# ai4ce/V2X-Sim

Measured on AMD Instinct MI355X. Metric: BEV frames/sec, V2VNet 5-agent detection (256x256 BEV), higher is better.
Workload: dtype bf16

## Files before the change

### v2x-sim_amd/csrc/conv_tail.hip

```cpp
#include "conv_stream.h"
#include <cstdlib>

typedef const __attribute__((address_space(1))) void *gptr_tl_t;
typedef __attribute__((address_space(3))) void *lptr_tl_t;

typedef unsigned int u32x2_tl_t __attribute__((ext_vector_type(2)));
typedef __attribute__((address_space(3))) u32x2_tl_t lds_u2_t;

static __device__ __attribute__((aligned(64))) unsigned int g_zero_page_tail[16];

struct TailArgs {
    const uint16_t *in;
    int in_cstride, in_coff;
    int N, H, W;
    const uint16_t *wA;
    const float *scA, *shA;
    int reluA;
    const uint16_t *wB;
    const float *scB, *shB;
    int reluB;
    const uint16_t *w2;
    const float *sc2, *sh2;
    int split;
    float *out, *out2;
    int out_cstride, out_coff, out2_cstride;
    int tiles_x, tiles_y, n_tiles;
    int xcd_walk;
};

namespace tail {
constexpr int TH = 8, TW = 32;
constexpr int MH = TH + 2, MW = TW + 2;
constexpr int IH = TH + 4, IW = TW + 4;
constexpr int NMID = MH * MW;
constexpr int WA_BYTES = 36 * 32 * 16;
constexpr int WB_BYTES = 36 * 64 * 16;
constexpr int IN_BYTES = IH * IW * 64;
constexpr int IN_PIECES = IN_BYTES / 1024;
constexpr int PPW = (IN_PIECES + 3) / 4;
constexpr int MID_BYTES = NMID * 64;
constexpr int GRP_BYTES = IN_BYTES + MID_BYTES;
constexpr int OFF_GRP = WA_BYTES + WB_BYTES;
constexpr int OFF_DUMMY = OFF_GRP + 2 * GRP_BYTES;
constexpr int OFF_TAB = OFF_DUMMY + 1024;
constexpr int SMEM = OFF_TAB + 288 * 4;
static_assert(IN_BYTES % 1024 == 0 && SMEM <= 160 * 1024, "LDS map");
__device__ __forceinline__ int swz4(int slot, int x) { return slot ^ ((x >> 1) & 3); }
}

__global__ __launch_bounds__(512) __attribute__((amdgpu_waves_per_eu(2, 2))) void conv3x3_tail_kernel(const TailArgs a) {
    using namespace tail;
    extern __shared__ __attribute__((aligned(16))) char smem[];
    const int tid = threadIdx.x;
    const int lane = tid & 63;
    const int wave8 = __builtin_amdgcn_readfirstlane(tid >> 6);
    const int grp = wave8 >> 2, wave = wave8 & 3;
    const int fj = lane & 15, fq = lane >> 4;
    char *s_wA = smem, *s_wB = smem + WA_BYTES;
    char *s_in = smem + OFF_GRP + grp * GRP_BYTES, *s_mid = s_in + IN_BYTES;

    for (int off = wave8 * 1024; off < WA_BYTES + WB_BYTES; off += 8192) {
        const char *src = off < WA_BYTES ? reinterpret_cast<const char *>(a.wA) + off : reinterpret_cast<const char *>(a.wB) + (off - WA_BYTES);
        __builtin_amdgcn_global_load_lds((gptr_tl_t)(src + lane * 16), (lptr_tl_t)(smem + off), 16, 0, 0);
    }
    bf16x8_t w2f[3][2];
#pragma unroll
    for (int i2 = 0; i2 < 3; ++i2)
#pragma unroll
        for (int s = 0; s < 2; ++s) w2f[i2][s] = *reinterpret_cast<const bf16x8_t *>(a.w2 + (size_t)(i2 * 16 + fj) * 64 + s * 32 + fq * 8);
    float *s_tab = reinterpret_cast<float *>(smem + OFF_TAB);
    for (int i = tid; i < 288; i += 512) {
        float v;
        if (i < 32) v = a.scA[i];
        else if (i < 64) v = a.shA[i - 32];
        else if (i < 128) v = a.scB[i - 64];
        else if (i < 192) v = a.shB[i - 128];
        else if (i < 240) v = a.sc2[i - 192];
        else v = a.sh2[i - 240];
        s_tab[i] = v;
    }
    const uint32_t floorA = a.reluA ? 0u : 0x80008000u, floorB = a.reluB ? 0u : 0x80008000u;
#pragma unroll
    for (int i = 0; i < 3; ++i) asm volatile("" ::"v"(w2f[i][0]), "v"(w2f[i][1]));

    const int r0 = wave < 2 ? 3 * wave : 6 + 2 * (wave - 2);
    int body_off[2][3];
#pragma unroll
    for (int sg = 0; sg < 2; ++sg)
#pragma unroll
        for (int kx = 0; kx < 3; ++kx) {
            const int col = 1 + 16 * sg + fj + kx;
            body_off[sg][kx] = (col * 4 + swz4(fq, col)) * 16;
        }
    int hr, hc, hvalid;
    {
        const int q = (wave == 3 ? 16 : 0) + fj;
        const int qc = q < 20 ? q : 19;
        hc = qc < 10 ? 0 : MW - 1;
        hr = qc < 10 ? qc : qc - 10;
        hvalid = (wave >= 2 && q < 20) ? 1 : 0;
    }
    const int txy = a.tiles_x * a.tiles_y;
    auto tile_coords = [&](int tile, int &n, int &ty, int &tx) {
        n = tile / txy;
        const int r = tile - n * txy;
        ty = r / a.tiles_x;
        tx = r - ty * a.tiles_x;
    };
    unsigned woff[PPW];
#pragma unroll
    for (int u = 0; u < PPW; ++u) {
        const int sidx = (wave + 4 * u) * 64 + lane;
        const int pix = sidx >> 2, phys = sidx & 3;
        const int pr = pix / IW, pcx = pix - pr * IW;
        woff[u] = (unsigned)(pr * a.W + pcx) * (unsigned)a.in_cstride + (unsigned)(swz4(phys, pcx) * 8);
    }
    auto load_window = [&](int tile) {
        int n, ty, tx;
        tile_coords(tile, n, ty, tx);
        const bool interior = ty > 0 && ty + 1 < a.tiles_y && tx > 0 && tx + 1 < a.tiles_x;
        if (interior) {
            const uint16_t *base = a.in + (size_t)((n * a.H + ty * TH - 2) * a.W + tx * TW - 2) * a.in_cstride + a.in_coff;
#pragma unroll
            for (int u = 0; u < PPW; ++u) {
                const int piece = wave + 4 * u;
                char *dst = piece < IN_PIECES ? s_in + piece * 1024 : smem + OFF_DUMMY;
                __builtin_amdgcn_global_load_lds((gptr_tl_t)(piece < IN_PIECES ? (const void *)(base + woff[u]) : (const void *)g_zero_page_tail), (lptr_tl_t)dst, 16, 0, 0);
            }
            return;
        }
        const int ln = fresh_lane();
#pragma unroll
        for (int u = 0; u < PPW; ++u) {
            const int piece = wave + 4 * u;
            const int sidx = piece * 64 + ln;
            const int pix = sidx >> 2, phys = sidx & 3;
            const int pr = pix / IW, pcx = pix - pr * IW;
            const int y = ty * TH - 2 + pr, x = tx * TW - 2 + pcx;
            const bool ok = piece < IN_PIECES && (unsigned)y < (unsigned)a.H && (unsigned)x < (unsigned)a.W;
            const unsigned off = (unsigned)((n * a.H + y) * a.W + x) * (unsigned)a.in_cstride + (unsigned)(a.in_coff + swz4(phys, pcx) * 8);
            char *dst = piece < IN_PIECES ? s_in + piece * 1024 : smem + OFF_DUMMY;
            __builtin_amdgcn_global_load_lds((gptr_tl_t)(ok ? (const void *)(a.in + off) : (const void *)g_zero_page_tail), (lptr_tl_t)dst, 16, 0, 0);
        }
    };

    const int n_pairs = (a.n_tiles + 1) >> 1;
    const v2x_tile_walk walk = v2x_xcd_tile_walk(n_pairs, a.xcd_walk);
    int pair_i = walk.first;
    {
        const int tile = 2 * pair_i + grp;
        if (pair_i < walk.end && tile < a.n_tiles) load_window(tile);
    }
    asm volatile("s_waitcnt vmcnt(0)" ::: "memory");
    __syncthreads();
    if (grp == 1) __builtin_amdgcn_s_barrier();

    for (; pair_i < walk.end; pair_i += walk.step) {
        const int tile = 2 * pair_i + grp;
        const bool has = tile < a.n_tiles;
        const int next_pair = pair_i + walk.step;
        const int next = 2 * next_pair + grp;
        const bool has_next = next_pair < walk.end && next < a.n_tiles;
        int n = 0, ty = 0, tx = 0;
        tile_coords(has ? tile : 0, n, ty, tx);

        if (has) {
            f32x4_t acc[6][2];
#pragma unroll
            for (int t = 0; t < 6; ++t)
#pragma unroll
                for (int i = 0; i < 2; ++i) acc[t][i] = (f32x4_t){0.f, 0.f, 0.f, 0.f};
            const char *wrow = s_in + r0 * (IW * 64);
#pragma unroll
            for (int kx = 0; kx < 3; ++kx) {
                bf16x8_t A[3][2], Bb[4][2], X[3];
#pragma unroll
                for (int ky = 0; ky < 3; ++ky)
#pragma unroll
                    for (int i = 0; i < 2; ++i) A[ky][i] = *reinterpret_cast<const bf16x8_t *>(s_wA + (((ky * 3 + kx) * 4 + fq) * 32 + i * 16 + fj) * 16);
#pragma unroll
                for (int rr = 0; rr < 4; ++rr)
#pragma unroll
                    for (int sg = 0; sg < 2; ++sg) Bb[rr][sg] = *reinterpret_cast<const bf16x8_t *>(wrow + rr * (IW * 64) + body_off[sg][kx]);
                if (wave < 2) {
#pragma unroll
                    for (int sg = 0; sg < 2; ++sg) X[sg] = *reinterpret_cast<const bf16x8_t *>(wrow + 4 * (IW * 64) + body_off[sg][kx]);
                    X[2] = X[1];
                } else {
                    const int col = hc + kx;
#pragma unroll
                    for (int ky = 0; ky < 3; ++ky) X[ky] = *reinterpret_cast<const bf16x8_t *>(s_in + (((hr + ky) * IW + col) * 4 + swz4(fq, col)) * 16);
                }
                __builtin_amdgcn_sched_barrier(0);
#pragma unroll
                for (int ky = 0; ky < 3; ++ky) {
#pragma unroll
                    for (int j = 0; j < 2; ++j)
#pragma unroll
                        for (int sg = 0; sg < 2; ++sg)
#pragma unroll
                            for (int i = 0; i < 2; ++i)
                                acc[2 * j + sg][i] = __builtin_amdgcn_mfma_f32_16x16x32_bf16(A[ky][i], Bb[j + ky][sg], acc[2 * j + sg][i], 0, 0, 0);
                    if (wave < 2) {
#pragma unroll
                        for (int sg = 0; sg < 2; ++sg)
#pragma unroll
                            for (int i = 0; i < 2; ++i)
                                acc[4 + sg][i] = __builtin_amdgcn_mfma_f32_16x16x32_bf16(A[ky][i], ky == 2 ? X[sg] : Bb[2 + ky][sg], acc[4 + sg][i], 0, 0, 0);
                    } else {
#pragma unroll
                        for (int i = 0; i < 2; ++i) acc[4][i] = __builtin_amdgcn_mfma_f32_16x16x32_bf16(A[ky][i], X[ky], acc[4][i], 0, 0, 0);
                    }
                }
                __builtin_amdgcn_sched_barrier(0);
            }
            float4 scA[2], shA[2];
#pragma unroll
            for (int i = 0; i < 2; ++i) {
                scA[i] = lds_ld4((lds_cf_t *)s_tab + i * 16 + fq * 4);
                shA[i] = lds_ld4((lds_cf_t *)s_tab + 32 + i * 16 + fq * 4);
            }
            auto emit = [&](const f32x4_t (&v)[2], int r, int c, bool keep, bool inside) __attribute__((always_inline)) {
#pragma unroll
                for (int i = 0; i < 2; ++i) {
                    uint2 o;
                    o.x = v2x_relu_bf16x2_floor(pack_bf16x2(v[i][0] * scA[i].x + shA[i].x, v[i][1] * scA[i].y + shA[i].y), floorA);
                    o.y = v2x_relu_bf16x2_floor(pack_bf16x2(v[i][2] * scA[i].z + shA[i].z, v[i][3] * scA[i].w + shA[i].w), floorA);
                    o.x = inside ? o.x : 0u;
                    o.y = inside ? o.y : 0u;
                    if (keep) *(lds_u2_t *)(s_mid + ((r * MW + c) * 4 + swz4(i * 2 + (fq >> 1), c)) * 16 + (fq & 1) * 8) = (u32x2_tl_t){o.x, o.y};
                }
            };
#pragma unroll
            for (int j = 0; j < 3; ++j) {
                if (j == 2 && wave >= 2) break;
                const int r = r0 + j;
                const int y = ty * TH - 1 + r;
                const bool inside = (unsigned)y < (unsigned)a.H;
#pragma unroll
                for (int sg = 0; sg < 2; ++sg) emit(acc[2 * j + sg], r, 1 + 16 * sg + fj, true, inside);
            }
            if (wave >= 2) {
                const int y = ty * TH - 1 + hr, x = tx * TW - 1 + hc;
                emit(acc[4], hr, hc, hvalid != 0, (unsigned)y < (unsigned)a.H && (unsigned)x < (unsigned)a.W);
            }
        }
        asm volatile("s_waitcnt lgkmcnt(0)" ::: "memory");
        __builtin_amdgcn_sched_barrier(0);
        __builtin_amdgcn_s_barrier();
        __builtin_amdgcn_sched_barrier(0);
        if (has_next) load_window(next);

        if (has) {
            f32x4_t acc[4][4];
#pragma unroll
            for (int i = 0; i < 4; ++i)
#pragma unroll
                for (int f = 0; f < 4; ++f) acc[i][f] = (f32x4_t){0.f, 0.f, 0.f, 0.f};
#pragma unroll
            for (int kx = 0; kx < 3; ++kx) {
                bf16x8_t A[2][4], B[8];
#pragma unroll
                for (int rr = 0; rr < 4; ++rr)
#pragma unroll
                    for (int ch = 0; ch < 2; ++ch) {
                        const int pr = 2 * wave + rr, pc = ch * 16 + fj + kx;
                        B[rr * 2 + ch] = *reinterpret_cast<const bf16x8_t *>(s_mid + ((pr * MW + pc) * 4 + swz4(fq, pc)) * 16);
                    }
#pragma unroll
                for (int i = 0; i < 4; ++i) A[0][i] = *reinterpret_cast<const bf16x8_t *>(s_wB + ((kx * 4 + fq) * 64 + i * 16 + fj) * 16);
#pragma unroll
                for (int ky = 0; ky < 3; ++ky) {
                    __builtin_amdgcn_sched_barrier(0);
                    if (ky < 2) {
#pragma unroll
                        for (int i = 0; i < 4; ++i)
                            A[(ky + 1) & 1][i] = *reinterpret_cast<const bf16x8_t *>(s_wB + ((((ky + 1) * 3 + kx) * 4 + fq) * 64 + i * 16 + fj) * 16);
                    }
                    __builtin_amdgcn_sched_barrier(0);
#pragma unroll
                    for (int i = 0; i < 4; ++i)
#pragma unroll
                        for (int f = 0; f < 4; ++f)
                            acc[i][f] = __builtin_amdgcn_mfma_f32_16x16x32_bf16(A[ky & 1][i], B[((f >> 1) + ky) * 2 + (f & 1)], acc[i][f], 0, 0, 0);
                }
                __builtin_amdgcn_sched_barrier(0);
            }
            float4 scB[4], shB[4], s2v[3], t2v[3];
#pragma unroll
            for (int i = 0; i < 4; ++i) {
                const int kappa = 32 * (i >> 1) + 8 * fq + 4 * (i & 1);
                scB[i] = lds_ld4((lds_cf_t *)s_tab + 64 + kappa);
                shB[i] = lds_ld4((lds_cf_t *)s_tab + 128 + kappa);
            }
#pragma unroll
            for (int i2 = 0; i2 < 3; ++i2) {
                s2v[i2] = lds_ld4((lds_cf_t *)s_tab + 192 + i2 * 16 + fq * 4);
                t2v[i2] = lds_ld4((lds_cf_t *)s_tab + 240 + i2 * 16 + fq * 4);
            }
#pragma unroll
            for (int f = 0; f < 4; ++f) {
                bf16x8_t hb[2];
#pragma unroll
                for (int s = 0; s < 2; ++s) {
                    float h[8];
#pragma unroll
                    for (int half = 0; half < 2; ++half) {
                        const int i = 2 * s + half;
                        h[half * 4 + 0] = acc[i][f][0] * scB[i].x + shB[i].x;
                        h[half * 4 + 1] = acc[i][f][1] * scB[i].y + shB[i].y;
                        h[half * 4 + 2] = acc[i][f][2] * scB[i].z + shB[i].z;
                        h[half * 4 + 3] = acc[i][f][3] * scB[i].w + shB[i].w;
                    }
                    uint4 p;
                    p.x = v2x_relu_bf16x2_floor(pack_bf16x2(h[0], h[1]), floorB);
                    p.y = v2x_relu_bf16x2_floor(pack_bf16x2(h[2], h[3]), floorB);
                    p.z = v2x_relu_bf16x2_floor(pack_bf16x2(h[4], h[5]), floorB);
                    p.w = v2x_relu_bf16x2_floor(pack_bf16x2(h[6], h[7]), floorB);
                    hb[s] = __builtin_bit_cast(bf16x8_t, p);
                }
                const int y = ty * TH + 2 * wave + (f >> 1), x = tx * TW + (f & 1) * 16 + fj;
                const uint32_t pix = (uint32_t)((n * a.H + y) * a.W + x);
                float *p1 = a.out + (size_t)pix * a.out_cstride + a.out_coff + fq * 4;
                float *p2 = a.out2 + (size_t)pix * a.out2_cstride + fq * 4 - a.split;
                float *p0 = (fq * 4 >= a.split) ? p2 : p1;
#pragma unroll
                for (int i2 = 0; i2 < 3; ++i2) {
                    f32x4_t d = (f32x4_t){0.f, 0.f, 0.f, 0.f};
#pragma unroll
                    for (int s = 0; s < 2; ++s) d = __builtin_amdgcn_mfma_f32_16x16x32_bf16(w2f[i2][s], hb[s], d, 0, 0, 0);
                    const float4 s2 = s2v[i2], t2 = t2v[i2];
                    const float v0 = d[0] * s2.x + t2.x, v1 = d[1] * s2.y + t2.y, v2 = d[2] * s2.z + t2.z, v3 = d[3] * s2.w + t2.w;
                    *reinterpret_cast<float4 *>(i2 == 0 ? p0 : p2 + i2 * 16) = make_float4(v0, v1, v2, v3);
                }
            }
        }
        if (has) asm volatile("s_waitcnt vmcnt(12)" ::: "memory");
        else asm volatile("s_waitcnt vmcnt(0)" ::: "memory");
        __builtin_amdgcn_sched_barrier(0);
        __builtin_amdgcn_s_barrier();
        __builtin_amdgcn_sched_barrier(0);
    }
    if (grp == 0) __builtin_amdgcn_s_barrier();
}


static int tail_launch(const TailArgs &a, hipStream_t s) {
    const int n_pairs = (a.n_tiles + 1) / 2;
    int grid = v2x_num_cus();
    if (grid > n_pairs) grid = n_pairs;
    return v2x_launch<conv3x3_tail_kernel>("conv3x3_tail_kernel", dim3(grid), dim3(512), tail::SMEM, s, a);
}

int v2x_conv_tail_dispatch(const v2x_conv_desc *first, const v2x_conv_desc *second, hipStream_t stream) {
    V2X_REQUIRE(first->ksize == 3 && first->stride == 1 && first->pad == 1 && first->w_layout == 1 && first->C0 == 32 && first->C1 == 0 && first->Cout == 32 &&
                    first->Cout2 == 0 && first->epilogue == V2X_EPI_BF16 && first->up0 == 0 && first->in_format == 0,
                "v2x_conv2d_pair (tail form): the first layer must be a halo-packed 3x3 stride-1 32 -> 32 bf16 layer on a bf16 NHWC input");
    V2X_REQUIRE(second->ksize == 3 && second->stride == 1 && second->pad == 1 && second->w_layout == 1 && second->C0 == 32 && second->C1 == 0 &&
                    second->Cout == 64 && second->Cout2 == 48 && second->epilogue == V2X_EPI_F32 && second->up0 == 0 && second->split > 0 &&
                    second->split % 4 == 0 && second->split <= 12 && second->relu2 == 0,
                "v2x_conv2d_pair (tail form): the second layer must be the fused heads (3x3 32 -> 64 chained with a 1x1 -> 48 without ReLU, fp32 outputs split at 4, 8 or 12 channels)");
    V2X_REQUIRE(first->in0 && first->weight && first->scale && first->shift && second->weight && second->scale && second->shift && second->weight2 &&
                    second->scale2 && second->shift2 && second->out && second->out2,
                "v2x_conv2d_pair (tail form): null pointer");
    V2X_REQUIRE(first->N == second->N && first->H == second->H && first->W == second->W, "v2x_conv2d_pair (tail form): extents differ");
    V2X_REQUIRE(first->N >= 0 && first->H > 0 && first->W > 0 && first->H % tail::TH == 0 && first->W % tail::TW == 0,
                "v2x_conv2d_pair (tail form): H %% 8 == 0 and W %% 32 == 0 required (H=%d W=%d)", first->H, first->W);
    V2X_REQUIRE((long long)first->N * first->H * first->W < (1ll << 27), "v2x_conv2d_pair (tail form): N*H*W must stay below 2^27 (32-bit element offsets)");
    V2X_REQUIRE(second->out_cstride >= second->split + second->out_coff && second->out_cstride % 4 == 0 && second->out_coff % 4 == 0 &&
                    second->out2_cstride >= 48 - second->split && second->out2_cstride % 4 == 0 && (reinterpret_cast<uintptr_t>(second->out) & 15) == 0 &&
                    (reinterpret_cast<uintptr_t>(second->out2) & 15) == 0,
                "v2x_conv2d_pair (tail form): bad output views (16-byte stores)");
    if (first->N == 0) return V2X_OK;
    TailArgs a;
    a.in = first->in0;
    a.in_cstride = 32;
    a.in_coff = 0;
    a.N = first->N;
    a.H = first->H;
    a.W = first->W;
    a.wA = first->weight;
    a.scA = first->scale;
    a.shA = first->shift;
    a.reluA = first->relu;
    a.wB = second->weight;
    a.scB = second->scale;
    a.shB = second->shift;
    a.reluB = second->relu;
    a.w2 = second->weight2;
    a.sc2 = second->scale2;
    a.sh2 = second->shift2;
    a.split = second->split;
    a.out = reinterpret_cast<float *>(second->out);
    a.out2 = reinterpret_cast<float *>(second->out2);
    a.out_cstride = second->out_cstride;
    a.out_coff = second->out_coff;
    a.out2_cstride = second->out2_cstride;
    a.tiles_x = a.W / tail::TW;
    a.tiles_y = a.H / tail::TH;
    a.n_tiles = a.N * a.tiles_x * a.tiles_y;
    a.xcd_walk = v2x_tune(V2X_TUNE_HALO_XCD);
    return tail_launch(a, stream);
}
```

Before: 6510.

## Walk vertical tile strips with a ring buffer to reuse fused-conv intermediate rows

The fused two-layer 3x3 tail kernel now walks whole vertical strips of tiles instead of independent 8x32 tiles. The intermediate (first-layer) rows sit in a rotating LDS ring, so each step loads and computes only 8 new input rows and 8 new mid rows rather than recomputing the 2-row halo. This removes redundant first-layer MFMA work and halo input loads. In exchange there is a priming step per strip and fewer independent work units (N*tiles_x strip pairs), which may reduce load balance across CUs.

```diff
diff --git a/v2x-sim_amd/csrc/conv_tail.hip b/v2x-sim_amd/csrc/conv_tail.hip
--- a/v2x-sim_amd/csrc/conv_tail.hip
+++ b/v2x-sim_amd/csrc/conv_tail.hip
@@ -31,12 +31,12 @@
 namespace tail {
 constexpr int TH = 8, TW = 32;
 constexpr int MH = TH + 2, MW = TW + 2;
-constexpr int IH = TH + 4, IW = TW + 4;
+constexpr int IH = TH + 2, IW = TW + 4;
 constexpr int NMID = MH * MW;
 constexpr int WA_BYTES = 36 * 32 * 16;
 constexpr int WB_BYTES = 36 * 64 * 16;
-constexpr int IN_BYTES = IH * IW * 64;
-constexpr int IN_PIECES = IN_BYTES / 1024;
+constexpr int IN_PIECES = (IH * IW * 64 + 1023) / 1024;
+constexpr int IN_BYTES = IN_PIECES * 1024;
 constexpr int PPW = (IN_PIECES + 3) / 4;
 constexpr int MID_BYTES = NMID * 64;
 constexpr int GRP_BYTES = IN_BYTES + MID_BYTES;
@@ -83,7 +83,7 @@
 #pragma unroll
     for (int i = 0; i < 3; ++i) asm volatile("" ::"v"(w2f[i][0]), "v"(w2f[i][1]));
 
-    const int r0 = wave < 2 ? 3 * wave : 6 + 2 * (wave - 2);
+    const int r0 = 2 + 2 * wave;
     int body_off[2][3];
 #pragma unroll
     for (int sg = 0; sg < 2; ++sg)
@@ -92,20 +92,10 @@
             const int col = 1 + 16 * sg + fj + kx;
             body_off[sg][kx] = (col * 4 + swz4(fq, col)) * 16;
         }
-    int hr, hc, hvalid;
-    {
-        const int q = (wave == 3 ? 16 : 0) + fj;
-        const int qc = q < 20 ? q : 19;
-        hc = qc < 10 ? 0 : MW - 1;
-        hr = qc < 10 ? qc : qc - 10;
-        hvalid = (wave >= 2 && q < 20) ? 1 : 0;
-    }
-    const int txy = a.tiles_x * a.tiles_y;
-    auto tile_coords = [&](int tile, int &n, int &ty, int &tx) {
-        n = tile / txy;
-        const int r = tile - n * txy;
-        ty = r / a.tiles_x;
-        tx = r - ty * a.tiles_x;
+    const int hc = fj < 8 ? 0 : MW - 1, hr = 2 + (fj & 7);
+    auto strip_coords = [&](int strip, int &n, int &tx) {
+        n = strip / a.tiles_x;
+        tx = strip - n * a.tiles_x;
     };
     unsigned woff[PPW];
 #pragma unroll
@@ -115,12 +105,12 @@
         const int pr = pix / IW, pcx = pix - pr * IW;
         woff[u] = (unsigned)(pr * a.W + pcx) * (unsigned)a.in_cstride + (unsigned)(swz4(phys, pcx) * 8);
     }
-    auto load_window = [&](int tile) {
-        int n, ty, tx;
-        tile_coords(tile, n, ty, tx);
-        const bool interior = ty > 0 && ty + 1 < a.tiles_y && tx > 0 && tx + 1 < a.tiles_x;
+    auto load_window = [&](int strip, int ty) {
+        int n, tx;
+        strip_coords(strip, n, tx);
+        const bool interior = ty >= 0 && ty + 1 < a.tiles_y && tx > 0 && tx + 1 < a.tiles_x;
         if (interior) {
-            const uint16_t *base = a.in + (size_t)((n * a.H + ty * TH - 2) * a.W + tx * TW - 2) * a.in_cstride + a.in_coff;
+            const uint16_t *base = a.in + (size_t)((n * a.H + ty * TH) * a.W + tx * TW - 2) * a.in_cstride + a.in_coff;
 #pragma unroll
             for (int u = 0; u < PPW; ++u) {
                 const int piece = wave + 4 * u;
@@ -136,41 +126,41 @@
             const int sidx = piece * 64 + ln;
             const int pix = sidx >> 2, phys = sidx & 3;
             const int pr = pix / IW, pcx = pix - pr * IW;
-            const int y = ty * TH - 2 + pr, x = tx * TW - 2 + pcx;
-            const bool ok = piece < IN_PIECES && (unsigned)y < (unsigned)a.H && (unsigned)x < (unsigned)a.W;
+            const int y = ty * TH + pr, x = tx * TW - 2 + pcx;
+            const bool ok = piece < IN_PIECES && pr < IH && (unsigned)y < (unsigned)a.H && (unsigned)x < (unsigned)a.W;
             const unsigned off = (unsigned)((n * a.H + y) * a.W + x) * (unsigned)a.in_cstride + (unsigned)(a.in_coff + swz4(phys, pcx) * 8);
             char *dst = piece < IN_PIECES ? s_in + piece * 1024 : smem + OFF_DUMMY;
             __builtin_amdgcn_global_load_lds((gptr_tl_t)(ok ? (const void *)(a.in + off) : (const void *)g_zero_page_tail), (lptr_tl_t)dst, 16, 0, 0);
         }
     };
 
-    const int n_pairs = (a.n_tiles + 1) >> 1;
+    const int n_strips = a.N * a.tiles_x;
+    const int n_pairs = (n_strips + 1) >> 1;
     const v2x_tile_walk walk = v2x_xcd_tile_walk(n_pairs, a.xcd_walk);
     int pair_i = walk.first;
-    {
-        const int tile = 2 * pair_i + grp;
-        if (pair_i < walk.end && tile < a.n_tiles) load_window(tile);
-    }
+    int ty = -1, ring = 2;
+    if (pair_i < walk.end && 2 * pair_i + grp < n_strips) load_window(2 * pair_i + grp, -1);
     asm volatile("s_waitcnt vmcnt(0)" ::: "memory");
     __syncthreads();
     if (grp == 1) __builtin_amdgcn_s_barrier();
 
-    for (; pair_i < walk.end; pair_i += walk.step) {
-        const int tile = 2 * pair_i + grp;
-        const bool has = tile < a.n_tiles;
-        const int next_pair = pair_i + walk.step;
-        const int next = 2 * next_pair + grp;
-        const bool has_next = next_pair < walk.end && next < a.n_tiles;
-        int n = 0, ty = 0, tx = 0;
-        tile_coords(has ? tile : 0, n, ty, tx);
+    while (pair_i < walk.end) {
+        const int strip = 2 * pair_i + grp;
+        const bool has = strip < n_strips;
+        const bool last = ty + 1 == a.tiles_y;
+        const int next_pair = last ? pair_i + walk.step : pair_i;
+        const int next_ty = last ? -1 : ty + 1;
+        const bool has_next = next_pair < walk.end && 2 * next_pair + grp < n_strips;
+        int n = 0, tx = 0;
+        strip_coords(has ? strip : 0, n, tx);
 
         if (has) {
-            f32x4_t acc[6][2];
-#pragma unroll
-            for (int t = 0; t < 6; ++t)
+            f32x4_t acc[5][2];
+#pragma unroll
+            for (int t = 0; t < 5; ++t)
 #pragma unroll
                 for (int i = 0; i < 2; ++i) acc[t][i] = (f32x4_t){0.f, 0.f, 0.f, 0.f};
-            const char *wrow = s_in + r0 * (IW * 64);
+            const char *wrow = s_in + (r0 - 2) * (IW * 64);
 #pragma unroll
             for (int kx = 0; kx < 3; ++kx) {
                 bf16x8_t A[3][2], Bb[4][2], X[3];
@@ -182,14 +172,10 @@
                 for (int rr = 0; rr < 4; ++rr)
 #pragma unroll
                     for (int sg = 0; sg < 2; ++sg) Bb[rr][sg] = *reinterpret_cast<const bf16x8_t *>(wrow + rr * (IW * 64) + body_off[sg][kx]);
-                if (wave < 2) {
-#pragma unroll
-                    for (int sg = 0; sg < 2; ++sg) X[sg] = *reinterpret_cast<const bf16x8_t *>(wrow + 4 * (IW * 64) + body_off[sg][kx]);
-                    X[2] = X[1];
-                } else {
+                if (wave == 3) {
                     const int col = hc + kx;
 #pragma unroll
-                    for (int ky = 0; ky < 3; ++ky) X[ky] = *reinterpret_cast<const bf16x8_t *>(s_in + (((hr + ky) * IW + col) * 4 + swz4(fq, col)) * 16);
+                    for (int ky = 0; ky < 3; ++ky) X[ky] = *reinterpret_cast<const bf16x8_t *>(s_in + (((hr - 2 + ky) * IW + col) * 4 + swz4(fq, col)) * 16);
                 }
                 __builtin_amdgcn_sched_barrier(0);
 #pragma unroll
@@ -201,13 +187,7 @@
 #pragma unroll
                             for (int i = 0; i < 2; ++i)
                                 acc[2 * j + sg][i] = __builtin_amdgcn_mfma_f32_16x16x32_bf16(A[ky][i], Bb[j + ky][sg], acc[2 * j + sg][i], 0, 0, 0);
-                    if (wave < 2) {
-#pragma unroll
-                        for (int sg = 0; sg < 2; ++sg)
-#pragma unroll
-                            for (int i = 0; i < 2; ++i)
-                                acc[4 + sg][i] = __builtin_amdgcn_mfma_f32_16x16x32_bf16(A[ky][i], ky == 2 ? X[sg] : Bb[2 + ky][sg], acc[4 + sg][i], 0, 0, 0);
-                    } else {
+                    if (wave == 3) {
 #pragma unroll
                         for (int i = 0; i < 2; ++i) acc[4][i] = __builtin_amdgcn_mfma_f32_16x16x32_bf16(A[ky][i], X[ky], acc[4][i], 0, 0, 0);
                     }
@@ -220,7 +200,7 @@
                 scA[i] = lds_ld4((lds_cf_t *)s_tab + i * 16 + fq * 4);
                 shA[i] = lds_ld4((lds_cf_t *)s_tab + 32 + i * 16 + fq * 4);
             }
-            auto emit = [&](const f32x4_t (&v)[2], int r, int c, bool keep, bool inside) __attribute__((always_inline)) {
+            auto emit = [&](const f32x4_t (&v)[2], int r, int c, bool inside) __attribute__((always_inline)) {
 #pragma unroll
                 for (int i = 0; i < 2; ++i) {
                     uint2 o;
@@ -228,30 +208,32 @@
                     o.y = v2x_relu_bf16x2_floor(pack_bf16x2(v[i][2] * scA[i].z + shA[i].z, v[i][3] * scA[i].w + shA[i].w), floorA);
                     o.x = inside ? o.x : 0u;
                     o.y = inside ? o.y : 0u;
-                    if (keep) *(lds_u2_t *)(s_mid + ((r * MW + c) * 4 + swz4(i * 2 + (fq >> 1), c)) * 16 + (fq & 1) * 8) = (u32x2_tl_t){o.x, o.y};
+                    *(lds_u2_t *)(s_mid + ((r * MW + c) * 4 + swz4(i * 2 + (fq >> 1), c)) * 16 + (fq & 1) * 8) = (u32x2_tl_t){o.x, o.y};
                 }
             };
-#pragma unroll
-            for (int j = 0; j < 3; ++j) {
-                if (j == 2 && wave >= 2) break;
-                const int r = r0 + j;
-                const int y = ty * TH - 1 + r;
+            const int slot0 = r0 + ring < MH ? r0 + ring : r0 + ring - MH;
+#pragma unroll
+            for (int j = 0; j < 2; ++j) {
+                const int y = ty * TH - 1 + r0 + j;
                 const bool inside = (unsigned)y < (unsigned)a.H;
 #pragma unroll
-                for (int sg = 0; sg < 2; ++sg) emit(acc[2 * j + sg], r, 1 + 16 * sg + fj, true, inside);
-            }
-            if (wave >= 2) {
+                for (int sg = 0; sg < 2; ++sg) emit(acc[2 * j + sg], slot0 + j, 1 + 16 * sg + fj, inside);
+            }
+            if (wave == 3) {
                 const int y = ty * TH - 1 + hr, x = tx * TW - 1 + hc;
-                emit(acc[4], hr, hc, hvalid != 0, (unsigned)y < (unsigned)a.H && (unsigned)x < (unsigned)a.W);
+                emit(acc[4], hr + ring < MH ? hr + ring : hr + ring - MH, hc, (unsigned)y < (unsigned)a.H && (unsigned)x < (unsigned)a.W);
             }
         }
         asm volatile("s_waitcnt lgkmcnt(0)" ::: "memory");
         __builtin_amdgcn_sched_barrier(0);
         __builtin_amdgcn_s_barrier();
         __builtin_amdgcn_sched_barrier(0);
-        if (has_next) load_window(next);
-
-        if (has) {
+        if (has_next) load_window(2 * next_pair + grp, next_ty);
+
+        const bool stage_b = has && ty >= 0;
+        if (stage_b) {
+            const int slotB0 = 2 * wave + ring < MH ? 2 * wave + ring : 2 * wave + ring - MH;
+            const int slotB2 = slotB0 + 2 < MH ? slotB0 + 2 : 0;
             f32x4_t acc[4][4];
 #pragma unroll
             for (int i = 0; i < 4; ++i)
@@ -264,7 +246,7 @@
                 for (int rr = 0; rr < 4; ++rr)
 #pragma unroll
                     for (int ch = 0; ch < 2; ++ch) {
-                        const int pr = 2 * wave + rr, pc = ch * 16 + fj + kx;
+                        const int pr = (rr < 2 ? slotB0 : slotB2) + (rr & 1), pc = ch * 16 + fj + kx;
                         B[rr * 2 + ch] = *reinterpret_cast<const bf16x8_t *>(s_mid + ((pr * MW + pc) * 4 + swz4(fq, pc)) * 16);
                     }
 #pragma unroll
@@ -335,18 +317,21 @@
                 }
             }
         }
-        if (has) asm volatile("s_waitcnt vmcnt(12)" ::: "memory");
+        if (stage_b) asm volatile("s_waitcnt vmcnt(12)" ::: "memory");
         else asm volatile("s_waitcnt vmcnt(0)" ::: "memory");
         __builtin_amdgcn_sched_barrier(0);
         __builtin_amdgcn_s_barrier();
         __builtin_amdgcn_sched_barrier(0);
+        pair_i = next_pair;
+        ty = next_ty;
+        ring = last ? 2 : (ring == 0 ? MH - 2 : ring - 2);
     }
     if (grp == 0) __builtin_amdgcn_s_barrier();
 }
 
 
 static int tail_launch(const TailArgs &a, hipStream_t s) {
-    const int n_pairs = (a.n_tiles + 1) / 2;
+    const int n_pairs = (a.N * a.tiles_x + 1) / 2;
     int grid = v2x_num_cus();
     if (grid > n_pairs) grid = n_pairs;
     return v2x_launch<conv3x3_tail_kernel>("conv3x3_tail_kernel", dim3(grid), dim3(512), tail::SMEM, s, a);
```

New measurement: 6560 (median of 6 runs). Within noise of the previous version (+0.8%).
